# clearml/clearml-serving

Measured on AMD Instinct MI355X. Metric: requests/sec + p50 latency, ResNet-50 & BERT-base dyn-batch, 1/2/4/8 MI355X, higher is better.
Workload: dtype bf16; 1 GPU; model=resnet50+bert-base, global_batch=512, seq_len=128, image=3x224x224, parallelism=dp1, max_batch_size=64, outputs_consumed=19494912

## Files before the change

### clearml_serving_amd/models/resnet.py

```python

import torch
import torch.nn as nn
import torch.nn.functional as F

from .. import ops
from . import register_arch


class FoldedConv(nn.Module):

    def __init__(self, cin, cout, k, stride=1, padding=0, relu=False):
        super().__init__()
        self.conv = nn.Conv2d(cin, cout, k, stride=stride, padding=padding,
                              bias=True)
        self.relu = relu

    def forward(self, x):
        c = self.conv
        if (c.kernel_size == (3, 3) and c.stride == (1, 1)
                and c.padding == (1, 1)
                and ops.conv3x3_supported(x, c.weight)):
            return ops.conv3x3_nhwc(x, c.weight, c.bias, relu=self.relu)
        y = c(x)
        if self.relu:
            y = F.relu(y)
        return y


class StemConv(nn.Module):

    def __init__(self, cin, cout, k, stride, padding, relu=True):
        super().__init__()
        self.conv = nn.Conv2d(cin, cout, k, stride=stride, padding=padding,
                              bias=True)
        self.relu = relu
        self.k, self.stride, self.padding = k, stride, padding

    def forward(self, x):
        if not x.is_cuda:
            y = self.conv(x)
            return F.relu(y) if self.relu else y
        n, c, h, w = x.shape
        oh = (h + 2 * self.padding - self.k) // self.stride + 1
        ow = (w + 2 * self.padding - self.k) // self.stride + 1
        cols = F.unfold(x.contiguous(), self.k, stride=self.stride,
                        padding=self.padding)
        flat = cols.transpose(1, 2).reshape(-1, c * self.k * self.k)
        wmat = self.conv.weight.reshape(self.conv.out_channels, -1)
        y = torch.nn.functional.linear(flat, wmat, self.conv.bias)
        if self.relu:
            y = torch.relu(y)
        return y.view(n, oh, ow, self.conv.out_channels) \
            .permute(0, 3, 1, 2)


def fold_bn_into_conv(conv: nn.Conv2d, bn: nn.BatchNorm2d) -> None:
    with torch.no_grad():
        inv_std = torch.rsqrt(bn.running_var + bn.eps)
        scale = bn.weight * inv_std
        conv.weight.mul_(scale[:, None, None, None])
        bias = conv.bias.data if conv.bias is not None else torch.zeros_like(bn.bias)
        conv.bias = nn.Parameter(bn.bias + (bias - bn.running_mean) * scale)


class Bottleneck(nn.Module):
    expansion = 4

    def __init__(self, cin, width, stride=1, downsample=None):
        super().__init__()
        cout = width * self.expansion
        self.conv1 = FoldedConv(cin, width, 1, relu=True)
        self.conv2 = FoldedConv(width, width, 3, stride=stride, padding=1,
                                relu=True)
        self.conv3 = FoldedConv(width, cout, 1, relu=False)
        self.downsample = downsample

    def forward(self, x):
        identity = x if self.downsample is None else self.downsample(x)
        y = self.conv1(x)
        y = self.conv2(y)
        y = self.conv3.conv(y)
        return ops.bias_relu_add(y, residual=identity)


class ResNet(nn.Module):
    def __init__(self, layers=(3, 4, 6, 3), num_classes=1000):
        super().__init__()
        self.stem = FoldedConv(3, 64, 7, stride=2, padding=3, relu=True)
        self.maxpool = nn.MaxPool2d(3, stride=2, padding=1)
        self.inplanes = 64
        self.layer1 = self._make_layer(64, layers[0], stride=1)
        self.layer2 = self._make_layer(128, layers[1], stride=2)
        self.layer3 = self._make_layer(256, layers[2], stride=2)
        self.layer4 = self._make_layer(512, layers[3], stride=2)
        self.fc = nn.Linear(512 * Bottleneck.expansion, num_classes)
        self._init_weights()

    def _make_layer(self, width, blocks, stride):
        downsample = None
        cout = width * Bottleneck.expansion
        if stride != 1 or self.inplanes != cout:
            downsample = FoldedConv(self.inplanes, cout, 1, stride=stride)
        layers = [Bottleneck(self.inplanes, width, stride, downsample)]
        self.inplanes = cout
        for _ in range(1, blocks):
            layers.append(Bottleneck(self.inplanes, width))
        return nn.Sequential(*layers)

    def _init_weights(self):
        for m in self.modules():
            if isinstance(m, nn.Conv2d):
                nn.init.kaiming_normal_(m.weight, mode="fan_out",
                                        nonlinearity="relu")
                if m.bias is not None:
                    nn.init.zeros_(m.bias)

    def forward(self, x):
        x = x.contiguous(memory_format=torch.channels_last)
        x = self.stem(x)
        x = self.maxpool(x)
        x = self.layer1(x)
        x = self.layer2(x)
        x = self.layer3(x)
        x = self.layer4(x)
        x = x.mean(dim=(2, 3))
        return self.fc(x)


@register_arch("resnet50")
def resnet50(num_classes: int = 1000) -> ResNet:
    return ResNet(layers=(3, 4, 6, 3), num_classes=num_classes).to(
        memory_format=torch.channels_last)


@register_arch("resnet101")
def resnet101(num_classes: int = 1000) -> ResNet:
    return ResNet(layers=(3, 4, 23, 3), num_classes=num_classes).to(
        memory_format=torch.channels_last)
```

### clearml_serving_amd/ops/__init__.py

```python

import importlib.machinery
import importlib.util
import math
import os
from typing import Optional, Tuple

import torch

_ext = None
_ext_error: Optional[str] = None
_FORCE_EAGER = os.environ.get("CLEARML_SERVING_AMD_FORCE_EAGER") == "1"


def _try_load_ext() -> None:
    global _ext, _ext_error
    if _ext is not None or _ext_error is not None:
        return
    so_path = os.path.join(os.path.dirname(__file__), "_hip_ops.so")
    if not os.path.exists(so_path):
        _ext_error = "extension not built ({} missing)".format(so_path)
        return
    try:
        loader = importlib.machinery.ExtensionFileLoader("_hip_ops", so_path)
        spec = importlib.util.spec_from_loader("_hip_ops", loader)
        mod = importlib.util.module_from_spec(spec)
        loader.exec_module(mod)
        _ext = mod
    except Exception as ex:
        _ext_error = "failed loading {}: {}".format(so_path, ex)


_try_load_ext()


def has_extension() -> bool:
    return _ext is not None


def _require_ext(opname: str):
    if _FORCE_EAGER:
        return None
    if _ext is None:
        raise RuntimeError(
            "clearml_serving_amd HIP extension required for GPU op '{}' but "
            "not loaded: {}. Build it with __graft_entry__.build() "
            "(hipcc --offload-arch=gfx950).".format(opname, _ext_error)
        )
    return _ext


def extension_or_none():
    return _ext


def layernorm(
    x: torch.Tensor, weight: torch.Tensor, bias: torch.Tensor,
    eps: float = 1e-5, residual: Optional[torch.Tensor] = None,
) -> torch.Tensor:
    if x.is_cuda:
        ext = _require_ext("layernorm")
        if ext is not None:
            return ext.layernorm(x, weight, bias, eps, residual)
    if residual is not None:
        x = x + residual
    return torch.nn.functional.layer_norm(
        x.float(), (x.shape[-1],), weight.float(), bias.float(), eps
    ).to(x.dtype)


def rmsnorm(
    x: torch.Tensor, weight: torch.Tensor, eps: float = 1e-6,
    residual: Optional[torch.Tensor] = None,
) -> torch.Tensor:
    if x.is_cuda:
        ext = _require_ext("rmsnorm")
        if ext is not None:
            return ext.rmsnorm(x, weight, eps, residual)
    xf = x.float()
    if residual is not None:
        xf = xf + residual.float()
        residual.copy_(xf.to(residual.dtype))
    out = xf * torch.rsqrt(xf.pow(2).mean(-1, keepdim=True) + eps)
    return (out * weight.float()).to(x.dtype)


def bias_gelu(x: torch.Tensor, bias: Optional[torch.Tensor] = None) -> torch.Tensor:
    if x.is_cuda:
        ext = _require_ext("bias_gelu")
        if ext is not None:
            return ext.bias_gelu(x, bias)
    if bias is not None:
        x = x + bias
    return torch.nn.functional.gelu(x.float()).to(x.dtype)


def bias_relu_add(
    x: torch.Tensor, bias: Optional[torch.Tensor] = None,
    residual: Optional[torch.Tensor] = None,
) -> torch.Tensor:
    if x.is_cuda:
        ext = _require_ext("bias_relu_add")
        if ext is not None:
            return ext.bias_relu_add(x, bias, residual)
    if bias is not None:
        x = x + bias
    if residual is not None:
        x = x + residual
    return torch.relu(x)


def silu_mul(gate: torch.Tensor, up: torch.Tensor) -> torch.Tensor:
    if gate.is_cuda:
        ext = _require_ext("silu_mul")
        if ext is not None:
            return ext.silu_mul(gate, up)
    return (torch.nn.functional.silu(gate.float()) * up.float()).to(gate.dtype)


F8_MAX = 448.0


def _quant_fp8_ref(y: torch.Tensor):
    y2 = y.float().reshape(-1, y.shape[-1])
    amax = y2.abs().amax(dim=1).clamp(min=1e-8)
    scale = (amax / F8_MAX).to(torch.float32)
    q = (y2 / scale[:, None]).clamp(-F8_MAX, F8_MAX).to(torch.float8_e4m3fn)
    return q.view(torch.uint8), scale


def rmsnorm_fp8(x: torch.Tensor, weight: torch.Tensor, eps: float = 1e-6,
                residual: Optional[torch.Tensor] = None):
    if x.is_cuda:
        ext = _require_ext("rmsnorm_fp8")
        if ext is not None:
            out8, scales = ext.rmsnorm_fp8(x, weight, eps, residual)
            return out8, scales
    return _quant_fp8_ref(rmsnorm(x, weight, eps, residual=residual))


def silu_mul_fp8(gate: torch.Tensor, up: torch.Tensor):
    if gate.is_cuda:
        ext = _require_ext("silu_mul_fp8")
        if ext is not None:
            out8, scales = ext.silu_mul_fp8(gate, up)
            return out8, scales
    return _quant_fp8_ref(silu_mul(gate, up))


def quant_fp8(x: torch.Tensor):
    if x.is_cuda:
        ext = _require_ext("quant_fp8")
        if ext is not None:
            out8, scales = ext.quant_fp8(x)
            return out8, scales
    return _quant_fp8_ref(x)


def swizzle_fp8_weight(w8: torch.Tensor) -> torch.Tensor:
    n, k = w8.shape
    assert k % 64 == 0
    v = w8.view(torch.uint8).reshape(n, k // 64, 2, 4, 8)
    return v.permute(0, 1, 3, 2, 4).contiguous().reshape(n, k)


def unswizzle_fp8_weight(w8s: torch.Tensor) -> torch.Tensor:
    n, k = w8s.shape
    v = w8s.view(torch.uint8).reshape(n, k // 64, 4, 2, 8)
    return v.permute(0, 1, 3, 2, 4).contiguous().reshape(n, k)


def skinny_gemm_fp8(a8: torch.Tensor, a_scale: torch.Tensor,
                    w8: torch.Tensor, w_scale: torch.Tensor,
                    swizzled: bool = False) -> torch.Tensor:
    if a8.is_cuda:
        ext = _require_ext("skinny_gemm_fp8")
        if ext is not None:
            ws = w8 if swizzled else swizzle_fp8_weight(w8)
            return ext.skinny_gemm_fp8(
                a8.view(torch.uint8), a_scale, ws.view(torch.uint8), w_scale)
    if swizzled:
        w8 = unswizzle_fp8_weight(w8)
    a = a8.view(torch.float8_e4m3fn).float() * a_scale[:, None]
    w = w8.view(torch.float8_e4m3fn).float() * w_scale[:, None]
    return (a @ w.t()).to(torch.bfloat16)


def skinny_gemm_fp8_v2(a8: torch.Tensor, a_scale: torch.Tensor,
                       w8: torch.Tensor, w_scale: torch.Tensor
                       ) -> torch.Tensor:
    if a8.is_cuda:
        ext = _require_ext("skinny_gemm_fp8_v2")
        if ext is not None:
            return ext.skinny_gemm_fp8_v2(
                a8.view(torch.uint8), a_scale, w8.view(torch.uint8), w_scale)
    a = a8.view(torch.float8_e4m3fn).float() * a_scale[:, None]
    w = w8.view(torch.float8_e4m3fn).float() * w_scale[:, None]
    return (a @ w.t()).to(torch.bfloat16)


def conv3x3_supported(x: torch.Tensor, w: torch.Tensor) -> bool:
    return (x.is_cuda and x.dtype == torch.bfloat16 and x.dim() == 4
            and x.shape[2] == x.shape[3] and x.shape[2] in (56, 28, 14)
            and x.shape[1] % 32 == 0 and w.shape[0] % 64 == 0
            and w.shape[2] == 3 and w.shape[3] == 3
            and os.environ.get("CMLS_CONV3", "1") != "0"
            and _ext is not None)


def conv3x3_nhwc(x: torch.Tensor, w: torch.Tensor,
                 bias: Optional[torch.Tensor] = None, relu: bool = False,
                 residual: Optional[torch.Tensor] = None) -> torch.Tensor:
    if (x.is_cuda and x.dtype == torch.bfloat16
            and x.shape[2] == x.shape[3] and x.shape[2] in (56, 28, 14)
            and x.shape[1] % 32 == 0 and w.shape[0] % 64 == 0):
        ext = _require_ext("conv3x3_nhwc")
        if ext is not None:
            xc = x.contiguous(memory_format=torch.channels_last)
            wc = w.contiguous(memory_format=torch.channels_last)
            return ext.conv3x3_nhwc(xc, wc, bias, relu, residual)
    y = torch.nn.functional.conv2d(x.float(), w.float(),
                                   bias.float() if bias is not None else None,
                                   stride=1, padding=1)
    if residual is not None:
        y = y + residual.float()
    if relu:
        y = torch.relu(y)
    return y.to(x.dtype)


def softmax(x: torch.Tensor, dim: int = -1) -> torch.Tensor:
    if x.is_cuda and dim in (-1, x.dim() - 1):
        ext = _require_ext("softmax")
        if ext is not None:
            return ext.softmax_lastdim(x)
    return torch.softmax(x.float(), dim=dim).to(x.dtype)


def attention(
    q: torch.Tensor, k: torch.Tensor, v: torch.Tensor,
    causal: bool = False, scale: Optional[float] = None,
    seq_lens: Optional[torch.Tensor] = None,
    layout: str = "bhsd",
) -> torch.Tensor:
    if scale is None:
        scale = 1.0 / math.sqrt(q.shape[-1])
    bshd = layout == "bshd"
    if q.is_cuda:
        ext = _require_ext("attention")
        if ext is not None:
            if os.environ.get("CMLS_ATTN_V2", "1") != "0":
                return ext.attention_prefill_v2(q, k, v, bool(causal),
                                                float(scale), seq_lens, bshd)
            return ext.attention_prefill(q, k, v, bool(causal), float(scale),
                                         seq_lens, bshd)
    if bshd:
        out = attention(q.permute(0, 2, 1, 3), k.permute(0, 2, 1, 3),
                        v.permute(0, 2, 1, 3), causal=causal, scale=scale,
                        seq_lens=seq_lens)
        return out.permute(0, 2, 1, 3).contiguous()
    qf, kf, vf = q.float(), k.float(), v.float()
    hq, hkv = q.shape[1], k.shape[1]
    if hkv != hq:
        rep = hq // hkv
        kf = kf.repeat_interleave(rep, dim=1)
        vf = vf.repeat_interleave(rep, dim=1)
    scores = torch.matmul(qf, kf.transpose(-1, -2)) * scale
    sq, sk = q.shape[2], k.shape[2]
    if causal:
        mask = torch.ones(sq, sk, dtype=torch.bool, device=q.device).tril(
            diagonal=sk - sq)
        scores = scores.masked_fill(~mask, float("-inf"))
    if seq_lens is not None:
        key_idx = torch.arange(sk, device=q.device)
        pad = key_idx[None, None, None, :] >= seq_lens[:, None, None, None]
        scores = scores.masked_fill(pad, float("-inf"))
    probs = torch.softmax(scores, dim=-1)
    return torch.matmul(probs, vf).to(q.dtype)


def _dequant_kv_cpu(cache: torch.Tensor, scale: torch.Tensor) -> torch.Tensor:
    f = cache.view(torch.float8_e4m3fn).float()
    return f * scale[..., None]


def attention_prefill_paged(
    q: torch.Tensor, k_cache: torch.Tensor, v_cache: torch.Tensor,
    block_table: torch.Tensor, kv_lens: torch.Tensor, q_lens: torch.Tensor,
    scale: Optional[float] = None,
    k_scale: Optional[torch.Tensor] = None,
    v_scale: Optional[torch.Tensor] = None,
) -> torch.Tensor:
    if scale is None:
        scale = 1.0 / math.sqrt(q.shape[-1])
    if q.is_cuda:
        ext = _require_ext("attention_prefill_paged")
        if ext is not None:
            if os.environ.get("CMLS_ATTN_V2", "1") != "0":
                return ext.attention_prefill_paged_v2(
                    q, k_cache, v_cache, block_table, kv_lens, q_lens,
                    float(scale), k_scale, v_scale)
            if k_scale is not None:
                raise RuntimeError("fp8 KV prefill needs the v2 kernel "
                                   "(CMLS_ATTN_V2=0 set?)")
            return ext.attention_prefill_paged(
                q, k_cache, v_cache, block_table, kv_lens, q_lens,
                float(scale))
    if k_scale is not None:
        return attention_prefill_paged(
            q, _dequant_kv_cpu(k_cache, k_scale),
            _dequant_kv_cpu(v_cache, v_scale), block_table, kv_lens, q_lens,
            scale)
    b, sq, h, d = q.shape
    hkv = k_cache.shape[1]
    bs = k_cache.shape[2]
    out = torch.zeros_like(q)
    for i in range(b):
        n = int(kv_lens[i])
        ql = int(q_lens[i])
        nb = (n + bs - 1) // bs
        blocks = block_table[i, :nb].long()
        k = k_cache[blocks].float().permute(1, 0, 2, 3).reshape(
            hkv, nb * bs, d)[:, :n]
        v = v_cache[blocks].float().permute(1, 0, 2, 3).reshape(
            hkv, nb * bs, d)[:, :n]
        o = attention(
            q[i, :ql].permute(1, 0, 2)[None].float(),
            k[None], v[None], causal=True, scale=scale)
        out[i, :ql] = o[0].permute(1, 0, 2).to(q.dtype)
    return out


def attention_decode(
    q: torch.Tensor, k_cache: torch.Tensor, v_cache: torch.Tensor,
    block_table: torch.Tensor, seq_lens: torch.Tensor,
    scale: Optional[float] = None,
    k_scale: Optional[torch.Tensor] = None,
    v_scale: Optional[torch.Tensor] = None,
) -> torch.Tensor:
    if scale is None:
        scale = 1.0 / math.sqrt(q.shape[-1])
    if q.is_cuda:
        ext = _require_ext("attention_decode")
        if ext is not None:
            return ext.attention_decode(q, k_cache, v_cache, block_table,
                                        seq_lens, float(scale),
                                        k_scale, v_scale)
    if k_scale is not None:
        return attention_decode(
            q, _dequant_kv_cpu(k_cache, k_scale),
            _dequant_kv_cpu(v_cache, v_scale), block_table, seq_lens, scale)
    bsz, hq, d = q.shape
    hkv = k_cache.shape[1]
    block_size = k_cache.shape[2]
    rep = hq // hkv
    out = torch.empty_like(q, dtype=q.dtype)
    qf = q.float()
    for b in range(bsz):
        n = int(seq_lens[b])
        nblocks = (n + block_size - 1) // block_size
        blocks = block_table[b, :nblocks].long()
        k = k_cache[blocks].float()
        v = v_cache[blocks].float()
        k = k.permute(1, 0, 2, 3).reshape(hkv, nblocks * block_size, d)[:, :n]
        v = v.permute(1, 0, 2, 3).reshape(hkv, nblocks * block_size, d)[:, :n]
        if rep > 1:
            k = k.repeat_interleave(rep, dim=0)
            v = v.repeat_interleave(rep, dim=0)
        scores = torch.einsum("hd,hnd->hn", qf[b], k) * scale
        probs = torch.softmax(scores, dim=-1)
        out[b] = torch.einsum("hn,hnd->hd", probs, v).to(q.dtype)
    return out


def kv_cache_write(
    k_new: torch.Tensor, v_new: torch.Tensor, k_cache: torch.Tensor,
    v_cache: torch.Tensor, slot_mapping: torch.Tensor,
    k_scale: Optional[torch.Tensor] = None,
    v_scale: Optional[torch.Tensor] = None,
) -> None:
    if k_new.is_cuda:
        ext = _require_ext("kv_cache_write")
        if ext is not None:
            ext.kv_cache_write(k_new, v_new, k_cache, v_cache, slot_mapping,
                               k_scale, v_scale)
            return
    block_size = k_cache.shape[2]
    fp8 = k_scale is not None
    for t in range(k_new.shape[0]):
        slot = int(slot_mapping[t])
        if slot < 0:
            continue
        blk, off = slot // block_size, slot % block_size
        if fp8:
            for cache, scales, new in ((k_cache, k_scale, k_new),
                                       (v_cache, v_scale, v_new)):
                row = new[t].float()
                amax = row.abs().amax(dim=-1).clamp_min(1e-8)
                sc = torch.exp2(torch.ceil(torch.log2(amax / 448.0)))
                q8 = (row / sc[:, None]).to(torch.float8_e4m3fn)
                cache[blk, :, off] = q8.view(torch.uint8)
                scales[blk, :, off] = sc
        else:
            k_cache[blk, :, off] = k_new[t]
            v_cache[blk, :, off] = v_new[t]


def rope_inplace(
    q: torch.Tensor, k: torch.Tensor, positions: torch.Tensor,
    theta: float = 10000.0,
) -> Tuple[torch.Tensor, torch.Tensor]:
    if q.is_cuda:
        ext = _require_ext("rope")
        if ext is not None:
            ext.rope_inplace(q, k, positions, float(theta))
            return q, k
    d = q.shape[-1]
    half = d // 2
    inv_freq = 1.0 / (theta ** (torch.arange(half, dtype=torch.float32,
                                             device=q.device) / half))
    angles = positions.float()[:, None] * inv_freq[None, :]
    cos = angles.cos()[:, None, :]
    sin = angles.sin()[:, None, :]
    for t in (q, k):
        tf = t.float().clone()
        lo, hi = tf[..., :half], tf[..., half:]
        t[..., :half] = (lo * cos - hi * sin).to(t.dtype)
        t[..., half:] = (hi * cos + lo * sin).to(t.dtype)
    return q, k


def sample_top_k_top_p(
    logits: torch.Tensor, temperature: float = 1.0, top_k: int = 0,
    top_p: float = 1.0, generator: Optional[torch.Generator] = None,
) -> torch.Tensor:
    if temperature == 0.0:
        return logits.argmax(dim=-1)
    if logits.is_cuda:
        ext = _require_ext("sample")
        if ext is not None:
            seed = int(torch.randint(0, 2**31 - 1, (1,),
                                     generator=generator).item())
            return ext.sample_top_k_top_p(
                logits, float(temperature), int(top_k), float(top_p), seed)
    lf = logits.float() / temperature
    if top_k and top_k < lf.shape[-1]:
        kth = torch.topk(lf, top_k, dim=-1).values[..., -1:]
        lf = lf.masked_fill(lf < kth, float("-inf"))
    if top_p < 1.0:
        sorted_logits, idx = torch.sort(lf, descending=True, dim=-1)
        probs = torch.softmax(sorted_logits, dim=-1)
        cutoff = probs.cumsum(dim=-1) > top_p
        cutoff[..., 0] = False
        sorted_logits = sorted_logits.masked_fill(cutoff, float("-inf"))
        lf = torch.full_like(lf, float("-inf")).scatter(-1, idx, sorted_logits)
    probs = torch.softmax(lf, dim=-1)
    return torch.multinomial(probs, 1, generator=generator).squeeze(-1)


def gemm_bf16(a: torch.Tensor, b: torch.Tensor) -> torch.Tensor:
    if a.is_cuda:
        ext = _require_ext("gemm_bf16")
        if ext is not None:
            m, k = a.shape
            n = b.shape[0]
            pm, pn, pk = (-m) % 128, (-n) % 128, (-k) % 32
            if pm or pn or pk:
                a2 = torch.nn.functional.pad(a, (0, pk, 0, pm))
                b2 = torch.nn.functional.pad(b, (0, pk, 0, pn))
                return ext.gemm_bf16(a2.contiguous(),
                                     b2.contiguous())[:m, :n].contiguous()
            return ext.gemm_bf16(a.contiguous(), b.contiguous())
    return (a.float() @ b.float().T).to(a.dtype)


def skinny_linear(x: torch.Tensor, weight: torch.Tensor) -> torch.Tensor:
    if (x.is_cuda and x.dtype == torch.bfloat16 and x.dim() == 2
            and x.shape[1] % 32 == 0 and weight.shape[0] % 16 == 0
            and os.environ.get("CMLS_SKINNY", "1") != "0"):
        m, k = x.shape
        n = weight.shape[0]
        if ((1 <= m <= 16 and n <= 8192 and k <= 8192)
                or (m <= 2 and n <= 8192)):
            ext = _require_ext("skinny_gemm")
            if ext is not None:
                return ext.skinny_gemm(x.contiguous(), weight, 1)
    return torch.nn.functional.linear(x, weight)
```

### clearml_serving_amd/ops/csrc/bindings.cpp

```cpp
#include <torch/extension.h>

torch::Tensor bias_relu_add(torch::Tensor x, c10::optional<torch::Tensor> bias,
                            c10::optional<torch::Tensor> residual);
torch::Tensor bias_gelu(torch::Tensor x, c10::optional<torch::Tensor> bias);
torch::Tensor silu_mul(torch::Tensor gate, torch::Tensor up);
torch::Tensor layernorm(torch::Tensor x, torch::Tensor weight,
                        torch::Tensor bias, double eps,
                        c10::optional<torch::Tensor> residual);
torch::Tensor rmsnorm(torch::Tensor x, torch::Tensor weight, double eps,
                      c10::optional<torch::Tensor> residual);
torch::Tensor softmax_lastdim(torch::Tensor x);
torch::Tensor attention_prefill(torch::Tensor q, torch::Tensor k,
                                torch::Tensor v, bool causal, double scale,
                                c10::optional<torch::Tensor> seq_lens,
                                bool bshd);
torch::Tensor sample_top_k_top_p(torch::Tensor logits, double temperature,
                                 long top_k, double top_p, long seed);
torch::Tensor attention_decode(torch::Tensor q, torch::Tensor k_cache,
                               torch::Tensor v_cache,
                               torch::Tensor block_table,
                               torch::Tensor seq_lens, double scale,
                               c10::optional<torch::Tensor> k_scale,
                               c10::optional<torch::Tensor> v_scale);
void kv_cache_write(torch::Tensor knew, torch::Tensor vnew,
                    torch::Tensor k_cache, torch::Tensor v_cache,
                    torch::Tensor slot_mapping,
                    c10::optional<torch::Tensor> k_scale,
                    c10::optional<torch::Tensor> v_scale);
torch::Tensor gemm_bf16(torch::Tensor a, torch::Tensor b);
torch::Tensor skinny_gemm(torch::Tensor a, torch::Tensor w, int64_t variant);
torch::Tensor attention_prefill_paged(torch::Tensor q, torch::Tensor k_cache,
                                      torch::Tensor v_cache,
                                      torch::Tensor block_table,
                                      torch::Tensor kv_lens,
                                      torch::Tensor q_lens, double scale);
void rope_inplace(torch::Tensor q, torch::Tensor k, torch::Tensor positions,
                  double theta);
std::vector<torch::Tensor> rmsnorm_fp8(torch::Tensor x, torch::Tensor weight,
                                       double eps,
                                       c10::optional<torch::Tensor> residual);
std::vector<torch::Tensor> silu_mul_fp8(torch::Tensor gate, torch::Tensor up);
std::vector<torch::Tensor> quant_fp8(torch::Tensor x);
torch::Tensor skinny_gemm_fp8(torch::Tensor a8, torch::Tensor a_scale,
                              torch::Tensor w8, torch::Tensor w_scale);
torch::Tensor skinny_gemm_fp8_v2(torch::Tensor a8, torch::Tensor a_scale,
                                 torch::Tensor w8, torch::Tensor w_scale);
torch::Tensor conv3x3_nhwc(torch::Tensor x, torch::Tensor w,
                           c10::optional<torch::Tensor> bias, bool relu,
                           c10::optional<torch::Tensor> residual);
torch::Tensor attention_prefill_v2(torch::Tensor q, torch::Tensor k,
                                   torch::Tensor v, bool causal, double scale,
                                   c10::optional<torch::Tensor> seq_lens,
                                   bool bshd, bool kdirect, bool pipe);
torch::Tensor attention_prefill_paged_v2(
    torch::Tensor q, torch::Tensor k_cache, torch::Tensor v_cache,
    torch::Tensor block_table, torch::Tensor kv_lens, torch::Tensor q_lens,
    double scale, c10::optional<torch::Tensor> k_scale,
    c10::optional<torch::Tensor> v_scale);

PYBIND11_MODULE(TORCH_EXTENSION_NAME, m) {
  m.doc() = "clearml-serving-amd gfx950 kernel library";
  m.def("bias_relu_add", &bias_relu_add, py::arg("x"),
        py::arg("bias") = py::none(), py::arg("residual") = py::none());
  m.def("bias_gelu", &bias_gelu, py::arg("x"), py::arg("bias") = py::none());
  m.def("silu_mul", &silu_mul);
  m.def("layernorm", &layernorm, py::arg("x"), py::arg("weight"),
        py::arg("bias"), py::arg("eps") = 1e-5,
        py::arg("residual") = py::none());
  m.def("rmsnorm", &rmsnorm, py::arg("x"), py::arg("weight"),
        py::arg("eps") = 1e-6, py::arg("residual") = py::none());
  m.def("softmax_lastdim", &softmax_lastdim);
  m.def("attention_prefill", &attention_prefill, py::arg("q"), py::arg("k"),
        py::arg("v"), py::arg("causal"), py::arg("scale"),
        py::arg("seq_lens") = py::none(), py::arg("bshd") = false);
  m.def("sample_top_k_top_p", &sample_top_k_top_p);
  m.def("rope_inplace", &rope_inplace);
  m.def("attention_decode", &attention_decode, py::arg("q"),
        py::arg("k_cache"), py::arg("v_cache"), py::arg("block_table"),
        py::arg("seq_lens"), py::arg("scale"),
        py::arg("k_scale") = py::none(), py::arg("v_scale") = py::none());
  m.def("kv_cache_write", &kv_cache_write, py::arg("knew"), py::arg("vnew"),
        py::arg("k_cache"), py::arg("v_cache"), py::arg("slot_mapping"),
        py::arg("k_scale") = py::none(), py::arg("v_scale") = py::none());
  m.def("gemm_bf16", &gemm_bf16);
  m.def("skinny_gemm", &skinny_gemm, py::arg("a"), py::arg("w"),
        py::arg("variant") = 0);
  m.def("attention_prefill_paged", &attention_prefill_paged);
  m.def("rmsnorm_fp8", &rmsnorm_fp8, py::arg("x"), py::arg("weight"),
        py::arg("eps") = 1e-6, py::arg("residual") = py::none());
  m.def("silu_mul_fp8", &silu_mul_fp8);
  m.def("quant_fp8", &quant_fp8);
  m.def("skinny_gemm_fp8", &skinny_gemm_fp8);
  m.def("skinny_gemm_fp8_v2", &skinny_gemm_fp8_v2);
  m.def("conv3x3_nhwc", &conv3x3_nhwc, py::arg("x"), py::arg("w"),
        py::arg("bias") = py::none(), py::arg("relu") = false,
        py::arg("residual") = py::none());
  m.def("attention_prefill_v2", &attention_prefill_v2, py::arg("q"),
        py::arg("k"), py::arg("v"), py::arg("causal"), py::arg("scale"),
        py::arg("seq_lens") = py::none(), py::arg("bshd") = false,
        py::arg("kdirect") = false, py::arg("pipe") = false);
  m.def("attention_prefill_paged_v2", &attention_prefill_paged_v2,
        py::arg("q"), py::arg("k_cache"), py::arg("v_cache"),
        py::arg("block_table"), py::arg("kv_lens"), py::arg("q_lens"),
        py::arg("scale"), py::arg("k_scale") = py::none(),
        py::arg("v_scale") = py::none());
}
```

Measured before the change: 13190 requests/s.

## Add MFMA conv1x1 NHWC kernel with fused bias, ReLU and residual for ResNet

Adds a custom HIP 1x1 convolution kernel built on bf16 MFMA that works directly on channels_last tensors and fuses bias, optional ReLU and an optional residual add into the epilogue. ResNet bottleneck 1x1 convs, including the strided downsample, are routed to it when their shape is in an allowlist. The final conv3 plus bias_relu_add pair becomes a single kernel. This removes a separate elementwise pass and the library conv dispatch. The kernel reads operands straight from global memory without LDS staging, so it may lose to the tuned library GEMM on the larger shapes.

```diff
diff --git a/clearml_serving_amd/models/resnet.py b/clearml_serving_amd/models/resnet.py
--- a/clearml_serving_amd/models/resnet.py
+++ b/clearml_serving_amd/models/resnet.py
@@ -15,8 +15,17 @@
                               bias=True)
         self.relu = relu
 
+    def routes_conv1x1(self, x):
+        c = self.conv
+        return (c.kernel_size == (1, 1) and c.padding == (0, 0)
+                and c.stride[0] == c.stride[1] and c.groups == 1
+                and ops.conv1x1_supported(x, c.weight, c.stride[0]))
+
     def forward(self, x):
         c = self.conv
+        if self.routes_conv1x1(x):
+            return ops.conv1x1_nhwc(x, c.weight, c.bias, relu=self.relu,
+                                    stride=c.stride[0])
         if (c.kernel_size == (3, 3) and c.stride == (1, 1)
                 and c.padding == (1, 1)
                 and ops.conv3x3_supported(x, c.weight)):
@@ -79,6 +88,10 @@
         identity = x if self.downsample is None else self.downsample(x)
         y = self.conv1(x)
         y = self.conv2(y)
+        if self.conv3.routes_conv1x1(y):
+            c = self.conv3.conv
+            return ops.conv1x1_nhwc(y, c.weight, c.bias, relu=True,
+                                    residual=identity)
         y = self.conv3.conv(y)
         return ops.bias_relu_add(y, residual=identity)
 
diff --git a/clearml_serving_amd/ops/__init__.py b/clearml_serving_amd/ops/__init__.py
--- a/clearml_serving_amd/ops/__init__.py
+++ b/clearml_serving_amd/ops/__init__.py
@@ -221,6 +221,54 @@
     y = torch.nn.functional.conv2d(x.float(), w.float(),
                                    bias.float() if bias is not None else None,
                                    stride=1, padding=1)
+    if residual is not None:
+        y = y + residual.float()
+    if relu:
+        y = torch.relu(y)
+    return y.to(x.dtype)
+
+
+_CONV1X1_ROUTED = frozenset({
+    (64, 64, 56, 1), (256, 64, 56, 1), (64, 256, 56, 1),
+    (256, 128, 56, 1), (512, 128, 28, 1), (128, 512, 28, 1),
+    (256, 512, 56, 2),
+    (512, 256, 28, 1), (1024, 256, 14, 1), (256, 1024, 14, 1),
+    (1024, 512, 14, 1), (2048, 512, 7, 1), (512, 2048, 7, 1),
+})
+
+
+def _conv1x1_kernel_ok(x: torch.Tensor, w: torch.Tensor, stride: int) -> bool:
+    return (x.is_cuda and x.dtype == torch.bfloat16 and x.dim() == 4
+            and w.dim() == 4 and w.shape[2] == 1 and w.shape[3] == 1
+            and x.shape[1] % 32 == 0 and w.shape[0] % 64 == 0
+            and stride in (1, 2))
+
+
+def conv1x1_supported(x: torch.Tensor, w: torch.Tensor,
+                      stride: int = 1) -> bool:
+    return (_conv1x1_kernel_ok(x, w, stride)
+            and x.shape[2] == x.shape[3]
+            and (x.shape[1], w.shape[0], x.shape[2], stride)
+            in _CONV1X1_ROUTED
+            and os.environ.get("CMLS_CONV1", "1") != "0"
+            and _ext is not None)
+
+
+def conv1x1_nhwc(x: torch.Tensor, w: torch.Tensor,
+                 bias: Optional[torch.Tensor] = None, relu: bool = False,
+                 residual: Optional[torch.Tensor] = None,
+                 stride: int = 1) -> torch.Tensor:
+    if _conv1x1_kernel_ok(x, w, stride):
+        ext = _require_ext("conv1x1_nhwc")
+        if ext is not None:
+            xc = x.contiguous(memory_format=torch.channels_last)
+            wc = w.contiguous()
+            rc = (residual.contiguous(memory_format=torch.channels_last)
+                  if residual is not None else None)
+            return ext.conv1x1_nhwc(xc, wc, bias, relu, rc, stride)
+    y = torch.nn.functional.conv2d(x.float(), w.float(),
+                                   bias.float() if bias is not None else None,
+                                   stride=stride)
     if residual is not None:
         y = y + residual.float()
     if relu:
diff --git a/clearml_serving_amd/ops/csrc/bindings.cpp b/clearml_serving_amd/ops/csrc/bindings.cpp
--- a/clearml_serving_amd/ops/csrc/bindings.cpp
+++ b/clearml_serving_amd/ops/csrc/bindings.cpp
@@ -48,6 +48,10 @@
 torch::Tensor conv3x3_nhwc(torch::Tensor x, torch::Tensor w,
                            c10::optional<torch::Tensor> bias, bool relu,
                            c10::optional<torch::Tensor> residual);
+torch::Tensor conv1x1_nhwc(torch::Tensor x, torch::Tensor w,
+                           c10::optional<torch::Tensor> bias, bool relu,
+                           c10::optional<torch::Tensor> residual,
+                           int64_t stride, int64_t pixel_tiles);
 torch::Tensor attention_prefill_v2(torch::Tensor q, torch::Tensor k,
                                    torch::Tensor v, bool causal, double scale,
                                    c10::optional<torch::Tensor> seq_lens,
@@ -95,6 +99,10 @@
   m.def("conv3x3_nhwc", &conv3x3_nhwc, py::arg("x"), py::arg("w"),
         py::arg("bias") = py::none(), py::arg("relu") = false,
         py::arg("residual") = py::none());
+  m.def("conv1x1_nhwc", &conv1x1_nhwc, py::arg("x"), py::arg("w"),
+        py::arg("bias") = py::none(), py::arg("relu") = false,
+        py::arg("residual") = py::none(), py::arg("stride") = 1,
+        py::arg("pixel_tiles") = 0);
   m.def("attention_prefill_v2", &attention_prefill_v2, py::arg("q"),
         py::arg("k"), py::arg("v"), py::arg("causal"), py::arg("scale"),
         py::arg("seq_lens") = py::none(), py::arg("bshd") = false,
diff --git a/clearml_serving_amd/ops/csrc/conv1x1.hip b/clearml_serving_amd/ops/csrc/conv1x1.hip
--- /dev/null
+++ b/clearml_serving_amd/ops/csrc/conv1x1.hip
@@ -0,0 +1,225 @@
+#include "common.h"
+
+namespace {
+
+typedef __attribute__((ext_vector_type(8))) short bf16x8_t;
+typedef __attribute__((ext_vector_type(4))) float f32x4_t;
+
+#define MFMA16(A, B, C) \
+  __builtin_amdgcn_mfma_f32_16x16x32_bf16((A), (B), (C), 0, 0, 0)
+
+constexpr int KSTEP = 32;
+constexpr int NWAVES = 4;
+constexpr int WAVE_N = 64;
+
+__device__ __forceinline__ float bf16_bits_to_f32(short v) {
+  return __uint_as_float(((unsigned int)(unsigned short)v) << 16);
+}
+
+template <int PT, int WN>
+__global__ __launch_bounds__(NWAVES * 64) void conv1x1_kernel(
+    const __hip_bfloat16* __restrict__ x,
+    const __hip_bfloat16* __restrict__ w,
+    const __hip_bfloat16* __restrict__ bias,
+    const __hip_bfloat16* __restrict__ residual,
+    __hip_bfloat16* __restrict__ out,
+    int M, int Cin, int Cout, int H, int W, int OH, int OW, int stride,
+    int relu) {
+  constexpr int WM = NWAVES / WN;
+  const int lane = threadIdx.x & 63;
+  const int wave = threadIdx.x >> 6;
+  const int wn = wave % WN;
+  const int wm = wave / WN;
+  const int frow = lane & 15;
+  const int g = lane >> 4;
+  const int fk = g * 8;
+
+  const int cout0 = (blockIdx.y * WN + wn) * WAVE_N;
+  const int pix0 = (blockIdx.x * WM + wm) * (PT * 16);
+  if (pix0 >= M) return;
+
+  const __hip_bfloat16* wrow[4];
+#pragma unroll
+  for (int t = 0; t < 4; ++t) {
+    const int c = cout0 + (t >> 1) * 32 + (frow >> 2) * 8 + (t & 1) * 4 +
+                  (frow & 3);
+    wrow[t] = w + (long)c * Cin + fk;
+  }
+  const __hip_bfloat16* xrow[PT];
+#pragma unroll
+  for (int pt = 0; pt < PT; ++pt) {
+    int p = pix0 + pt * 16 + frow;
+    p = p < M ? p : M - 1;
+    long row = p;
+    if (stride != 1) {
+      const int ow = p % OW;
+      const int t2 = p / OW;
+      const int oh = t2 % OH;
+      const int n = t2 / OH;
+      row = ((long)n * H + (long)oh * stride) * W + (long)ow * stride;
+    }
+    xrow[pt] = x + row * Cin + fk;
+  }
+
+  f32x4_t acc[4][PT];
+#pragma unroll
+  for (int t = 0; t < 4; ++t)
+#pragma unroll
+    for (int pt = 0; pt < PT; ++pt) acc[t][pt] = f32x4_t{0.f, 0.f, 0.f, 0.f};
+
+  bf16x8_t wf[2][4], xf[2][PT];
+  auto load_frags = [&](int buf, int k0) {
+#pragma unroll
+    for (int t = 0; t < 4; ++t)
+      wf[buf][t] = *reinterpret_cast<const bf16x8_t*>(wrow[t] + k0);
+#pragma unroll
+    for (int pt = 0; pt < PT; ++pt)
+      xf[buf][pt] = *reinterpret_cast<const bf16x8_t*>(xrow[pt] + k0);
+  };
+  auto compute = [&](int buf) {
+#pragma unroll
+    for (int pt = 0; pt < PT; ++pt)
+#pragma unroll
+      for (int t = 0; t < 4; ++t)
+        acc[t][pt] = MFMA16(wf[buf][t], xf[buf][pt], acc[t][pt]);
+  };
+
+  load_frags(0, 0);
+  for (int k0 = 0; k0 < Cin; k0 += 2 * KSTEP) {
+    const bool has1 = k0 + KSTEP < Cin;
+    if (has1) load_frags(1, k0 + KSTEP);
+    compute(0);
+    if (has1) {
+      if (k0 + 2 * KSTEP < Cin) load_frags(0, k0 + 2 * KSTEP);
+      compute(1);
+    }
+  }
+
+  float bv[2][8];
+#pragma unroll
+  for (int h = 0; h < 2; ++h) {
+#pragma unroll
+    for (int e = 0; e < 8; ++e)
+      bv[h][e] = bias ? to_f32(bias[cout0 + h * 32 + g * 8 + e]) : 0.f;
+  }
+#pragma unroll
+  for (int pt = 0; pt < PT; ++pt) {
+    const int p = pix0 + pt * 16 + frow;
+    if (p >= M) continue;
+#pragma unroll
+    for (int h = 0; h < 2; ++h) {
+      const long off = (long)p * Cout + cout0 + h * 32 + g * 8;
+      float v[8];
+#pragma unroll
+      for (int e = 0; e < 8; ++e)
+        v[e] = acc[h * 2 + (e >> 2)][pt][e & 3] + bv[h][e];
+      if (residual) {
+        const bf16x8_t r8 =
+            *reinterpret_cast<const bf16x8_t*>(residual + off);
+#pragma unroll
+        for (int e = 0; e < 8; ++e) v[e] += bf16_bits_to_f32(r8[e]);
+      }
+      bf16x8 o;
+#pragma unroll
+      for (int e = 0; e < 8; ++e) {
+        const float r = relu ? fmaxf(v[e], 0.f) : v[e];
+        o.h[e] = __float2bfloat16(r);
+      }
+      *reinterpret_cast<uint32x4*>(out + off) = o.u;
+    }
+  }
+}
+
+}
+
+#ifndef CMLS_KERNEL_ONLY
+torch::Tensor conv1x1_nhwc(torch::Tensor x, torch::Tensor w,
+                           c10::optional<torch::Tensor> bias, bool relu,
+                           c10::optional<torch::Tensor> residual,
+                           int64_t stride, int64_t pixel_tiles) {
+  TORCH_CHECK(x.dim() == 4 && w.dim() == 4, "conv1x1: 4-D tensors");
+  TORCH_CHECK(x.is_cuda() && w.is_cuda() && x.device() == w.device(),
+              "conv1x1: x and w must be on the same GPU");
+  TORCH_CHECK(x.scalar_type() == at::kBFloat16 &&
+              w.scalar_type() == at::kBFloat16, "conv1x1: bf16 only");
+  TORCH_CHECK(x.is_contiguous(at::MemoryFormat::ChannelsLast),
+              "conv1x1: x must be channels_last");
+  TORCH_CHECK(stride == 1 || stride == 2, "conv1x1: stride must be 1 or 2");
+  const long N = x.size(0), Cin = x.size(1), H = x.size(2), W = x.size(3);
+  const long Cout = w.size(0);
+  TORCH_CHECK(w.size(1) == Cin && w.size(2) == 1 && w.size(3) == 1,
+              "conv1x1: weight must be [Cout, Cin, 1, 1]");
+  TORCH_CHECK(w.stride(0) == Cin && w.stride(1) == 1,
+              "conv1x1: weight rows must be dense [Cout, Cin]");
+  TORCH_CHECK(Cin % KSTEP == 0, "conv1x1: Cin % 32 != 0");
+  TORCH_CHECK(Cout % WAVE_N == 0, "conv1x1: Cout % 64 != 0");
+  TORCH_CHECK(N > 0 && H > 0 && W > 0, "conv1x1: empty input");
+  const long OH = (H - 1) / stride + 1, OW = (W - 1) / stride + 1;
+  const long M = N * OH * OW;
+  TORCH_CHECK(M < (1L << 31), "conv1x1: too many output pixels");
+
+  auto out = torch::empty_strided(
+      {N, Cout, OH, OW},
+      {OH * OW * Cout, 1, OW * Cout, Cout}, x.options());
+  const __hip_bfloat16* bp = nullptr;
+  if (bias.has_value() && bias->defined()) {
+    TORCH_CHECK(bias->scalar_type() == at::kBFloat16 &&
+                bias->device() == x.device(), "conv1x1: bias bf16, same GPU");
+    TORCH_CHECK(bias->is_contiguous() && bias->numel() == Cout,
+                "conv1x1: bias must be contiguous [Cout]");
+    bp = (const __hip_bfloat16*)bias->data_ptr();
+  }
+  const __hip_bfloat16* rp = nullptr;
+  if (residual.has_value() && residual->defined()) {
+    TORCH_CHECK(residual->scalar_type() == at::kBFloat16 &&
+                residual->device() == x.device(),
+                "conv1x1: residual bf16, same GPU");
+    TORCH_CHECK(residual->sizes() == out.sizes(),
+                "conv1x1: residual must have the output shape");
+    TORCH_CHECK(residual->is_contiguous(at::MemoryFormat::ChannelsLast),
+                "conv1x1: residual must be channels_last");
+    rp = (const __hip_bfloat16*)residual->data_ptr();
+  }
+  TORCH_CHECK(((uintptr_t)x.data_ptr() | (uintptr_t)w.data_ptr() |
+               (uintptr_t)rp | (uintptr_t)out.data_ptr()) % 16 == 0,
+              "conv1x1: x, w, residual must be 16-byte aligned");
+  hipStream_t stream_ = cmls::current_stream();
+
+  const int WN = (Cout % 256 == 0) ? 4 : (Cout % 128 == 0) ? 2 : 1;
+  const int WM = NWAVES / WN;
+  const long ny = Cout / (WN * WAVE_N);
+  TORCH_CHECK(pixel_tiles == 0 || pixel_tiles == 1 || pixel_tiles == 2 ||
+              pixel_tiles == 4, "conv1x1: pixel_tiles must be 0, 1, 2 or 4");
+  int PT = (int)pixel_tiles;
+  if (PT == 0) {
+    PT = 1;
+    for (int cand : {4, 2}) {
+      const long bm = (long)cand * 16 * WM;
+      if (((M + bm - 1) / bm) * ny >= 128) { PT = cand; break; }
+    }
+  }
+  const long BM = (long)PT * 16 * WM;
+  dim3 grid((unsigned)((M + BM - 1) / BM), (unsigned)ny);
+  dim3 block(NWAVES * 64);
+
+#define LAUNCH_C1(PT_, WN_)                                                 \
+  hipLaunchKernelGGL((conv1x1_kernel<PT_, WN_>), grid, block, 0, stream_,   \
+                     (const __hip_bfloat16*)x.data_ptr(),                   \
+                     (const __hip_bfloat16*)w.data_ptr(), bp, rp,           \
+                     (__hip_bfloat16*)out.data_ptr(), (int)M, (int)Cin,     \
+                     (int)Cout, (int)H, (int)W, (int)OH, (int)OW,           \
+                     (int)stride, relu ? 1 : 0)
+#define LAUNCH_C1_PT(PT_)                                                   \
+  do {                                                                      \
+    if (WN == 4) LAUNCH_C1(PT_, 4);                                         \
+    else if (WN == 2) LAUNCH_C1(PT_, 2);                                    \
+    else LAUNCH_C1(PT_, 1);                                                 \
+  } while (0)
+  if (PT == 4) LAUNCH_C1_PT(4);
+  else if (PT == 2) LAUNCH_C1_PT(2);
+  else LAUNCH_C1_PT(1);
+#undef LAUNCH_C1_PT
+#undef LAUNCH_C1
+  return out;
+}
+#endif
```

New measurement: 13140 requests/s. Within noise of the previous version (-0.4%).
